# zifeo/distributed-sgd

Hardware: NVIDIA H100
Metric: sgd_samples_per_sec (higher is better)
Workload: dtype f64

## Files before the change

### distributed_sgd_b200/csrc/dsgd_api.cu

```cuda
#include "../../include/dsgd.h"

#include <cuda.h>
#include <cuda_runtime.h>
#include <dlfcn.h>
#include <nccl.h>

#include <algorithm>
#include <cmath>
#include <cstdarg>
#include <cstdio>
#include <cstring>
#include <limits>
#include <mutex>
#include <string>
#include <type_traits>
#include <utility>
#include <vector>

#include "dsgd_kernels.cuh"
#include "dsgd_persistent.cuh"
#include "dsgd_stream.cuh"
#include "dsgd_async.cuh"
#include "dsgd_metrics.cuh"
#include "dsgd_calibrate.cuh"
// ... 91 lines not shown
  dev_buf<float> yabs;
  dev_buf<double> sw;

  dev_buf<double> w, g, d, w_req;
  dev_buf<float> w32, w32_req;
  dev_buf<unsigned long long> n_exact;
  bool stream_ready = false;
  dev_buf<double> scal;
  dev_buf<unsigned long long> cnt;
  dev_buf<double> partial;
  dev_buf<double> out2;
  dev_buf<double> cls_out;
  dev_buf<double> gsum;
  std::vector<int32_t> worker_counts;
  int32_t n_local = 1, k_total = 0;
  bool have_d = false;

  dev_buf<int32_t> samples;
  int64_t samples_n = 0;
  dev_buf<double> losses;
  dev_buf<double> lrs;
  dev_buf<double> preds;
  dev_buf<int32_t> eval_ids;
  dev_buf<unsigned long long> m_keys, m_alt, m_cnt;
  dev_buf<unsigned char> m_tmp;
  dev_buf<double> m_val, m_valt;
  dev_buf<limb_sum> c_pre;
  dev_buf<unsigned long long> c_cnt, c_merged;
  dev_buf<int> c_excl;
  dev_buf<double> c_thr;
  dev_buf<long long> c_tp, c_fp;
  dev_buf<double> k_score, k_cw;
  dev_buf<int8_t> k_lab;
  dev_buf<unsigned long long> k_ctl, k_eval;
  int k_fit_occ = 0;
  int k_fit_occ_w = 0;
  dev_buf<int> i_hull;
  dev_buf<u256> i_wpt;
  dev_buf<int> i_wkeep;
  dev_buf<double> i_wthr, i_wblk;
  dev_buf<double> i_out, i_map;
  dev_buf<long long> i_blk;
  dev_buf<unsigned long long> i_ctl;

  ncclComm_t comm = nullptr;

  dev_buf<double> p_wbuf[2];
  dev_buf<double> p_gbuf[3];
  dev_buf<double2> p_rec[3];
  dev_buf<unsigned long long> p_acc;
  dev_buf<unsigned> p_hinge;
  dev_buf<unsigned long long> p_hcode;
  dev_buf<double> p_loss_nrm;
  dev_buf<unsigned> p_bar;
  bool p_ready = false;
  dev_buf<long long> p_tl;

  dev_buf<double> avg;
  bool avg_on = false;
  int64_t avg_n = 0;

  owned_stream astream;
  owned_stream stream2;
  dev_buf<double> m_w;
  dev_buf<double> outbox;
  peer_ptr peer_w[kMaxReplicas];
  dev_buf<int> a_stop;
  dev_buf<unsigned long long> a_cnt;
  dev_buf<double> a_scratch;
  dev_buf<int32_t> a_rows, a_assigned, a_replay;
  dev_buf<int32_t> u_idx; dev_buf<double> u_val;
  std::mutex u_mu;
  bool a_running = false;
  owned_event a_ev0, a_ev1;

  dev_buf<double> xblk;
  peer_ptr peer_x[kMaxWorld];
  int grid_limit = 0;
  int64_t x_step = 0;
  int64_t x_steps_run = 0;
  dev_buf<unsigned long long> x_llw;
  dev_buf<unsigned long long> x_stats;

  int32_t prof_every = 0;
  int64_t prof_seen = 0;
  std::vector<std::pair<owned_event, owned_event>> prof_events;
  size_t prof_used = 0;

  mutable std::string err;
  mutable std::string info;
};

static thread_local std::string g_create_err;

struct nccl_api {
  ncclResult_t (*GetUniqueId)(ncclUniqueId *) = nullptr;
  ncclResult_t (*CommInitRank)(ncclComm_t *, int, ncclUniqueId, int) = nullptr;
  ncclResult_t (*AllReduce)(const void *, void *, size_t, ncclDataType_t, ncclRedOp_t, ncclComm_t, cudaStream_t) = nullptr;
  ncclResult_t (*CommDestroy)(ncclComm_t) = nullptr;
  const char *(*GetErrorString)(ncclResult_t) = nullptr;
  bool ok = false;
  std::string why;
};
static nccl_api &nccl() {
  static nccl_api api = [] {
    nccl_api a;
// ... 1943 lines not shown
  memcpy(id, &u, sizeof u);
  return DSGD_OK;
}

extern "C" int dsgd_comm_init(dsgd_ctx *ctx, const uint8_t id[DSGD_UNIQUE_ID_BYTES]) {
  if (!ctx) return DSGD_ERR_INVALID;
  NEED(id, DSGD_ERR_INVALID, "dsgd_comm_init: id is NULL");
  NEED(!ctx->comm, DSGD_ERR_STATE, "dsgd_comm_init: communicator already initialised");
  CU(cudaSetDevice(ctx->device));
  ncclUniqueId u;
  memcpy(&u, id, sizeof u);
  NEED(nccl().ok, DSGD_ERR_NCCL, "%s", nccl().why.c_str());
  NC(nccl().CommInitRank(&ctx->comm, ctx->world, u, ctx->rank));
  return DSGD_OK;
}

constexpr int kPCons = 8, kPUpd = 6, kPStages = 8, kPStagePairs = 2560, kPMaxChunks = 128;
using PSmem = PersistSmem<kPCons, kPUpd, kPStages, kPStagePairs, kPMaxChunks>;
constexpr int kPersistForms = 28, kPersistFused = 24;
constexpr bool pf_multi(int f) { return f >= kPersistFused; }
constexpr int pf_weight(int f) { return pf_multi(f) ? kUnweighted : f / 8; }
constexpr bool pf_l1(int f) { return (f & 4) != 0; }
template <int... F>
static void *const *persist_forms(std::integer_sequence<int, F...>) {
  static void *const k[] = {(void *)k_sync_persistent<kPCons, kPUpd, kPStages, kPStagePairs, kPMaxChunks, pf_multi(F),
                                                      (F & 2) != 0, (F & 1) != 0, pf_l1(F), pf_weight(F)>...};
  return k;
}
static void *const *const kPersistKernels = persist_forms(std::make_integer_sequence<int, kPersistForms>{});
static int persist_form(bool multi, bool avg, bool lr_table, bool l1, int weight) {
  if (multi) return kPersistFused + 2 * avg + lr_table;
  return 8 * weight + 4 * l1 + 2 * avg + lr_table;
}
static size_t persist_smem(int f) {
  return sizeof(PSmem) + (pf_weight(f) == kSampleWeighted ? sizeof(PersistSwSmem<kPStages>) : 0);
}
static bool persist_timeline() { static const bool v = getenv("DSGD_PERSIST_TIMELINE") != nullptr; return v; }

static int persist_prepare(dsgd_ctx *ctx, int64_t n_steps) {
  if (!ctx->p_ready) {
    const int64_t nv = (int64_t)ctx->dim + 2;
    const size_t vd = sizeof(double) * (size_t)nv;
    for (int i = 0; i < 2; ++i) CU(ctx->p_wbuf[i].alloc(nv));
    for (int i = 0; i < 3; ++i) {
      CU(ctx->p_gbuf[i].alloc(nv));
      CU(cudaMemsetAsync(ctx->p_gbuf[i], 0, vd, ctx->stream));
      CU(ctx->p_rec[i].alloc(nv));
      CU(cudaMemsetAsync(ctx->p_rec[i], 0, 2 * vd, ctx->stream));
    }
    CU(ctx->p_acc.alloc(3 * kAccStride));
    CU(ctx->p_bar.alloc(4));
    for (int f = 0; f < kPersistForms; ++f)
      CU(cudaFuncSetAttribute(kPersistKernels[f], cudaFuncAttributeMaxDynamicSharedMemorySize, (int)persist_smem(f)));
    ctx->p_ready = true;
  }
  int rc = ctx->p_hinge.grow(ctx, (int64_t)ctx->sm_count * n_steps, 4096 * (int64_t)ctx->sm_count);
  if (rc) return rc;
  if (weighting(ctx) == kSampleWeighted &&
      (rc = ctx->p_hcode.grow(ctx, (int64_t)ctx->sm_count * n_steps, 4096 * (int64_t)ctx->sm_count)))
    return rc;
  return ctx->p_loss_nrm.grow(ctx, 2 * n_steps, 2 * 4096);
}

static int persist_grid(const dsgd_ctx *ctx, int64_t batch) {
  const int g = ctx->grid_limit > 0 ? std::min(ctx->grid_limit, ctx->sm_count) : ctx->sm_count;
  if (cdiv(batch, kMaxRowsPerCta) > g) return 0;
  if (ctx->n_pairs >= (1ll << 31)) return 0;
  return g;
}
static bool persist_multi_fits(const dsgd_ctx *ctx, int G) {
  const int slice = (cdiv(ctx->dim + 1, G) + 31) & ~31;
  return slice <= (kPCons + kPUpd) * 32;
}

static cudaError_t persist_launch(dsgd_ctx *ctx, int form, int G, void **args) {
  void *fn = kPersistKernels[form];
  const size_t smem = persist_smem(form);
  if (ctx->grid_limit > 0) return cudaLaunchKernel(fn, dim3(G), dim3((kPCons + kPUpd + 1) * 32), args, smem, ctx->stream);
  return cudaLaunchCooperativeKernel(fn, dim3(G), dim3((kPCons + kPUpd + 1) * 32), args, smem, ctx->stream);
}

static size_t xblk_stride(const dsgd_ctx *ctx) { return (size_t)(ctx->dim + kReplicaPad); }
static size_t xblk_words(const dsgd_ctx *ctx) { return ((size_t)ctx->dim + 1 + 31) / 32; }
static size_t xblk_bm_offset(const dsgd_ctx *ctx) { return 2 * (size_t)kMaxWorld * 2 * xblk_stride(ctx); }
static size_t xblk_doubles(const dsgd_ctx *ctx) { return xblk_bm_offset(ctx) + (size_t)kMaxWorld * 2 * xblk_words(ctx); }

static int xblk_ensure(dsgd_ctx *ctx) {
  if (ctx->xblk) return DSGD_OK;
  CU(cudaSetDevice(ctx->device));
  CU(ctx->xblk.alloc((int64_t)xblk_doubles(ctx)));
  CU(cudaMemset(ctx->xblk, 0, sizeof(double) * xblk_doubles(ctx)));
  CU(ctx->x_stats.alloc(4));
  CU(cudaMemset(ctx->x_stats, 0, sizeof(unsigned long long) * 4));
  return DSGD_OK;
}

static int xllw_ensure(dsgd_ctx *ctx) {
  if (ctx->x_llw) return DSGD_OK;
  CU(ctx->x_llw.alloc(2 * 2 * (int64_t)xblk_stride(ctx)));
  CU(cudaMemsetAsync(ctx->x_llw, 0, 2 * 2 * sizeof(unsigned long long) * xblk_stride(ctx), ctx->stream));
  return DSGD_OK;
}

static bool xchg_complete(const dsgd_ctx *ctx) {
  if (ctx->world <= 1 || ctx->world > kMaxWorld || !ctx->xblk) return false;
  for (int r = 0; r < ctx->world; ++r)
    if (r != ctx->rank && !ctx->peer_x[r]) return false;
  return true;
}

static int persist_run(dsgd_ctx *ctx, bool multi, const int32_t *samples_dev, int64_t n_per_step, int64_t n_steps,
                       double lr, const double *lrs_host, double *losses_dev) {
  int rc = persist_prepare(ctx, n_steps);
  if (rc) return rc;
  const int G = persist_grid(ctx, n_per_step);
  NEED((uint64_t)G * (uint64_t)(n_steps + 2) < (1ull << 32), DSGD_ERR_INVALID, "dsgd_sync_steps: too many steps for one launch");
  PersistParams pp;
  memset(&pp, 0, sizeof pp);
  pp.rp16 = ctx->rp16; pp.pairs = ctx->pairs; pp.label = ctx->label; pp.samples = samples_dev;
  pp.n_steps = n_steps; pp.batch = (int32_t)n_per_step; pp.dim = ctx->dim;
  pp.wbuf[0] = ctx->p_wbuf[0]; pp.wbuf[1] = ctx->p_wbuf[1];
  for (int i = 0; i < 3; ++i) { pp.gbuf[i] = ctx->p_gbuf[i]; pp.rec[i] = ctx->p_rec[i]; }
  pp.d = ctx->d; pp.acc = ctx->p_acc; pp.bar = ctx->p_bar; pp.hinge = ctx->p_hinge; pp.losses = losses_dev;
  pp.loss_nrm = ctx->p_loss_nrm;
  pp.w_out = ctx->w; pp.w32_out = ctx->w32; pp.scal = ctx->scal;
  pp.abort_flag = reinterpret_cast<int *>(ctx->p_bar + 1);
  CU(cudaMemsetAsync(ctx->p_acc, 0, sizeof(unsigned long long) * 3 * kAccStride, ctx->stream));
  pp.lambda = ctx->lambda; pp.lr = lr; pp.world = 1;
  CU(cudaMemsetAsync(ctx->p_bar, 0, sizeof(unsigned) * 4, ctx->stream));
  if (persist_timeline()) {
    if (!ctx->p_tl) CU(ctx->p_tl.alloc(kTlWords));
    CU(cudaMemsetAsync(ctx->p_tl, 0, sizeof(long long) * kTlWords, ctx->stream));
    pp.tl = ctx->p_tl;
  }
  if (!multi) {
    k_rec_init<<<cdiv(ctx->dim, 256), 256, 0, ctx->stream>>>(ctx->w, ctx->dim, ctx->p_rec[0], ctx->p_rec[1], ctx->p_rec[2]);
    LAUNCHED();
    pp.k_den = 1.0;
    pp.timeout_cycles = 4000000000ll;
  } else {
    CU(cudaMemcpyAsync(ctx->p_wbuf[0], ctx->w, sizeof(double) * (size_t)ctx->dim, cudaMemcpyDeviceToDevice, ctx->stream));
    pp.k_den = (double)ctx->world;
    pp.timeout_cycles = 20000000000ll;
    pp.world = ctx->world; pp.rank = ctx->rank; pp.step_base = ctx->x_step;
    pp.xstride = (int)xblk_stride(ctx);
    pp.xwords = (int)xblk_words(ctx);
    for (int r = 0; r < ctx->world; ++r) {
      unsigned long long *blk = reinterpret_cast<unsigned long long *>((r == ctx->rank) ? ctx->xblk.p : ctx->peer_x[r].p);
      pp.xval[r] = blk;
      pp.xbm[r] = blk + xblk_bm_offset(ctx);
    }
    if ((rc = xllw_ensure(ctx))) return rc;
    pp.llw[0] = ctx->x_llw;
    pp.llw[1] = ctx->x_llw + 2 * xblk_stride(ctx);
    pp.xstats = ctx->x_stats;
  }
  if (ctx->avg_on) pp.avg = ctx->avg;
  if (lrs_host) {
    if ((rc = ctx->lrs.grow(ctx, n_steps, 1024))) return rc;
    CU(cudaMemcpyAsync(ctx->lrs, lrs_host, sizeof(double) * (size_t)n_steps, cudaMemcpyHostToDevice, ctx->stream));
    pp.lrs = ctx->lrs;
    pp.lr = 0.0;
  }
  void *args[] = {&pp};
  const bool l1 = !multi && ctx->lambda1 > 0.0;
  pp.lambda1 = l1 ? ctx->lambda1 : 0.0;
  pp.w_pos = ctx->cw_pos; pp.w_neg = ctx->cw_neg;
  const int weight = multi ? kUnweighted : weighting(ctx);
  if (weight == kSampleWeighted) { pp.sw = ctx->sw; pp.hcode = ctx->p_hcode; }
  const int form = persist_form(multi, ctx->avg_on, lrs_host != nullptr, l1, weight);
  cudaError_t launch_err = cudaSuccess;
  profiled(ctx, [&] { launch_err = persist_launch(ctx, form, G, args); });
  CU(launch_err);
  LAUNCHED();
  if (ctx->avg_on) ctx->avg_n += n_steps;
  if (multi) {
    ctx->x_step += n_steps + 6;
    ctx->x_steps_run += n_steps;
  }
  return DSGD_OK;
}

extern "C" int dsgd_reserve(dsgd_ctx *ctx, int64_t n_samples, int64_t n_steps) {
  if (!ctx) return DSGD_ERR_INVALID;
  NEED(n_samples >= 0 && n_steps >= 0, DSGD_ERR_INVALID, "dsgd_reserve: negative size");
  CU(cudaSetDevice(ctx->device));
  int rc = ctx->samples.grow(ctx, n_samples, 1024);
  if (rc) return rc;
  if ((rc = ctx->losses.grow(ctx, n_steps, 1024))) return rc;
  if ((rc = ctx->lrs.grow(ctx, n_steps, 1024))) return rc;
// ... 679 lines not shown
```

### distributed_sgd_b200/csrc/dsgd_persistent.cuh

```cuda
#pragma once
#include <cuda_runtime.h>
#include <stdint.h>

#include <type_traits>

#include "dsgd_fixed.cuh"
#include "dsgd_kernels.cuh"

namespace dsgd {

constexpr int kMaxWorld = 8;

struct PersistParams {
  const uint32_t *rp16;
  const uint2 *pairs;
  const int8_t *label;
  const int32_t *samples;
  int64_t n_steps;
  int32_t batch;
  int32_t dim;
  double *wbuf[2];
  double *gbuf[3];
  double2 *rec[3];
  const double *d;
  unsigned long long *acc;
  unsigned *hinge;
  double *losses;
  double *w_out;
  float *w32_out;
  double *scal;
  unsigned *bar;
  int *abort_flag;
  double lambda, lr, k_den;
  long long timeout_cycles;
  long long *tl;
  int world, rank;
  int64_t step_base;
  unsigned long long *xval[kMaxWorld];
  unsigned long long *xbm[kMaxWorld];
  int xstride, xwords;
  unsigned long long *llw[2];
  unsigned long long *xstats;
  double *avg;
  const double *lrs;
  double lambda1;
  double *loss_nrm;
  double w_pos, w_neg;
  const double *sw;
  unsigned long long *hcode;
};
static_assert(sizeof(PersistParams) <= 4000, "kernel parameter space is 4 KB");

__device__ __forceinline__ uint32_t smem_u32(const void *p) { return (uint32_t)__cvta_generic_to_shared(p); }
__device__ __forceinline__ void mbar_init(uint64_t *b, unsigned count) {
  asm volatile("mbarrier.init.shared::cta.b64 [%0], %1;" ::"r"(smem_u32(b)), "r"(count) : "memory");
}
__device__ __forceinline__ void mbar_expect_tx(uint64_t *b, unsigned bytes) {
  asm volatile("mbarrier.arrive.expect_tx.shared::cta.b64 _, [%0], %1;" ::"r"(smem_u32(b)), "r"(bytes) : "memory");
}
__device__ __forceinline__ void mbar_arrive(uint64_t *b) {
  asm volatile("mbarrier.arrive.shared::cta.b64 _, [%0];" ::"r"(smem_u32(b)) : "memory");
}
__device__ __forceinline__ void bulk_g2s(void *dst, const void *src, unsigned bytes, uint64_t *b) {
  asm volatile("cp.async.bulk.shared::cluster.global.mbarrier::complete_tx::bytes [%0], [%1], %2, [%3];" ::"r"(
                   smem_u32(dst)),
               "l"(src), "r"(bytes), "r"(smem_u32(b))
               : "memory");
}
__device__ __forceinline__ bool mbar_try_wait(uint64_t *b, unsigned parity) {
  unsigned ok;
  asm volatile(
      "{\n\t.reg .pred p;\n\tmbarrier.try_wait.parity.shared::cta.b64 p, [%1], %2;\n\tselp.u32 %0, 1, 0, p;\n\t}"
      : "=r"(ok)
      : "r"(smem_u32(b)), "r"(parity)
      : "memory");
  return ok != 0;
}
__device__ __forceinline__ void mbar_wait(uint64_t *b, unsigned parity, int *abort_flag, long long timeout) {
  if (mbar_try_wait(b, parity)) return;
  const long long t0 = clock64();
  unsigned spins = 0;
  while (!mbar_try_wait(b, parity)) {
    if ((++spins & 255u) == 0u && (clock64() - t0 > timeout || *(volatile int *)abort_flag)) {
      *(volatile int *)abort_flag = 1;
      return;
    }
  }
}
__device__ __forceinline__ unsigned ld_relaxed_gpu(const unsigned *p) {
  unsigned v;
  asm volatile("ld.relaxed.gpu.global.u32 %0, [%1];" : "=r"(v) : "l"(p) : "memory");
  return v;
}
__device__ __forceinline__ void red_release_gpu_add(unsigned *p, unsigned v) {
  asm volatile("red.release.gpu.global.add.u32 [%0], %1;" ::"l"(p), "r"(v) : "memory");
}
__device__ __forceinline__ unsigned atom_acq_rel_gpu_add(unsigned *p, unsigned v) {
  unsigned old;
  asm volatile("atom.acq_rel.gpu.global.add.u32 %0, [%1], %2;" : "=r"(old) : "l"(p), "r"(v) : "memory");
  return old;
}
__device__ __forceinline__ void st_relaxed_gpu(unsigned *p, unsigned v) {
// ... 18 lines not shown
  const unsigned long long w1 = (bits >> 32) | ((unsigned long long)tag << 32);
  asm volatile("st.relaxed.sys.global.v2.u64 [%0], {%1, %2};" ::"l"(dst), "l"(w0), "l"(w1) : "memory");
}
__device__ __forceinline__ bool ll_try_load(const unsigned long long *src, unsigned tag, double &v) {
  unsigned long long w0, w1;
  asm volatile("ld.relaxed.sys.global.v2.u64 {%0, %1}, [%2];" : "=l"(w0), "=l"(w1) : "l"(src) : "memory");
  if ((unsigned)(w0 >> 32) != tag || (unsigned)(w1 >> 32) != tag) return false;
  v = __longlong_as_double((long long)((w0 & 0xffffffffull) | (w1 << 32)));
  return true;
}
__device__ __forceinline__ void ll_store32(unsigned long long *dst, unsigned v, unsigned tag) {
  const unsigned long long w = (unsigned long long)v | ((unsigned long long)tag << 32);
  asm volatile("st.relaxed.sys.global.u64 [%0], %1;" ::"l"(dst), "l"(w) : "memory");
}
__device__ __forceinline__ bool ll_try_load32(const unsigned long long *src, unsigned tag, unsigned &v) {
  unsigned long long w;
  asm volatile("ld.relaxed.sys.global.u64 %0, [%1];" : "=l"(w) : "l"(src) : "memory");
  v = (unsigned)w;
  return (unsigned)(w >> 32) == tag;
}

__device__ __forceinline__ double apply_update(double wv, double graw, double c, bool add_c, double k_den, double lr) {
  double v = filt(graw);
  if (v != 0.0) {
    if (add_c) v = filt(v + c);
    if (v != 0.0) {
      const double mean = (k_den == 1.0) ? v : filt(v / k_den);
      const double step = filt(mean * lr);
      wv = filt(wv - step);
    }
  }
  return wv;
}

__device__ __forceinline__ bool grid_barrier_arrive_wait(unsigned *bar, unsigned target, int *abort_flag, long long timeout) {
  red_release_gpu_add(bar, 1u);
  const long long t0 = clock64();
  unsigned spins = 0;
  bool ok = true;
  while ((int)(ld_relaxed_gpu(bar) - target) < 0) {
    if ((++spins & 1023u) == 0u && (clock64() - t0 > timeout || *(volatile int *)abort_flag)) {
      *(volatile int *)abort_flag = 1;
      ok = false;
      break;
    }
  }
  return ok;
}

constexpr int kChunkPairs = 128;
static_assert(kChunkPairs == kFoldPairs, "a listed row's chunks are the chunks of the row fold");
constexpr uint32_t kChunkGlobal = 1u << 31;
constexpr int kMaxRowsPerCta = 32;
constexpr int kRowBarFirst = 5, kRowBars = 11;

template <int kMaxChunks>
struct StageMeta {
  int n_rows;
  int n_chunks;
  int n_multi;
  int two_pass;
  int n_pairs;
  int row_y[kMaxRowsPerCta];
  uint32_t row_b[kMaxRowsPerCta];
  int row_len[kMaxRowsPerCta];
  short row_first[kMaxRowsPerCta];
  short row_nch[kMaxRowsPerCta];
  signed char row_bar[kMaxRowsPerCta];
  uint32_t ch_off[kMaxChunks];
  short ch_n[kMaxChunks];
  short ch_row[kMaxChunks];
  double part[kMaxChunks];
};

template <int kStages>
struct PersistSwSmem {
  double row_c[kStages][kMaxRowsPerCta];
  unsigned long long code;
};

template <int kCons, int kUpd, int kStages, int kStagePairs, int kMaxChunks>
struct PersistSmem {
  uint2 ring[kStages][kStagePairs];
  StageMeta<kMaxChunks> meta[kStages];
  uint64_t full[kStages];
  uint64_t empty[kStages];
  uint64_t c_bar[2];
  uint64_t u_bar;
  double red[kCons + kUpd][2];
  double c_val[2];
  double nrm_val[2];
  unsigned hinge_acc;
  int ok;
  long long tl_warp[kCons + kUpd];
};

#define DSGD_TL(slot_)                                                                        \
  do {                                                                                        \
    if (p.tl && blockIdx.x == 0 && lane == 0 && t < 256) p.tl[t * 16 + (slot_)] = clock64(); \
  } while (0)
constexpr int kTlSteps = 4, kTlFirst = 100, kTlCtas = 160, kTlPerCta = 4;
constexpr int kTlWords = 256 * 16 + kTlSteps * kTlCtas * kTlPerCta;

template <bool kL1 = false>
struct FetchLocal {
  const double2 *R;
  uint64_t *cbar;
  unsigned cpar;
  const double *cval;
  int *abort_flag;
  long long timeout;
  double k_den, lr;
  double tau = 0.0;
  double c = 0.0;
  bool add_c = false, have_c = false, good = true;
  __device__ __forceinline__ void need_c() {
    if (!have_c) {
      mbar_wait(cbar, cpar, abort_flag, timeout);
      c = *(volatile const double *)cval;
      add_c = (c != 0.0) && (fabs(c) > kEps);
      have_c = true;
// ... 55 lines not shown
        w0[u] = 0ull; w1[u] = 0ull;
        if (pend & (1u << u))
          asm volatile("ld.relaxed.sys.global.v2.u64 {%0, %1}, [%2];" : "=l"(w0[u]), "=l"(w1[u]) : "l"(LW + 2 * (size_t)pr[u].x) : "memory");
      }
#pragma unroll
      for (int u = 0; u < 4; ++u)
        if ((pend & (1u << u)) && (unsigned)(w0[u] >> 32) == tag && (unsigned)(w1[u] >> 32) == tag) {
          wv[u] = __longlong_as_double((long long)((w0[u] & 0xffffffffull) | (w1[u] << 32)));
          pend &= ~(1u << u);
        }
      if (pend && (++spins & 63u) == 0u && (clock64() - t0 > timeout || *(volatile int *)abort_flag)) {
        *(volatile int *)abort_flag = 1;
        good = false;
        pend = 0;
      }
    }
  }
  __device__ __forceinline__ double get1(uint32_t col) {
    double v;
    spin(LW + 2 * (size_t)col, v);
    return v;
  }
};

template <int kMaxChunks>
__device__ __forceinline__ void chunk_pairs(const StageMeta<kMaxChunks> &mt, const uint2 *ring, const uint2 *pairs, int c, int lane,
                                            uint2 (&pr)[4]) {
  const uint32_t off = mt.ch_off[c];
  const int n = mt.ch_n[c];
  const uint2 *src = (off & kChunkGlobal) ? (pairs + (off & ~kChunkGlobal)) : (ring + off);
#pragma unroll
  for (int u = 0; u < 4; ++u) {
    const int k = u * 32 + lane;
    pr[u] = (k < n) ? src[k] : make_uint2(0u, 0u);
  }
}

template <int kCons, int kMaxChunks, int kWeight = kUnweighted, class Fetch>
__device__ __forceinline__ std::conditional_t<kWeight == kSampleWeighted, unsigned long long, unsigned> consume_stage(
    StageMeta<kMaxChunks> &mt, const uint2 *ring, const uint2 *pairs, double *gbase, const int gstride, Fetch &fetch, int warp,
    int lane, long long *tl, const uint2 (*pre)[4] = nullptr, double w_pos = 1.0, double w_neg = 1.0,
    const double *row_c = nullptr) {
  using Hinge = std::conditional_t<kWeight == kSampleWeighted, unsigned long long, unsigned>;
  const int n_ch = mt.n_chunks;
  Hinge hinge = 0;
  auto scale_of = [&](int yi, double y, int m) {
    if constexpr (kWeight == kSampleWeighted) return yi > 0 ? row_c[m] : -row_c[m];
    return kWeight == kClassWeighted ? (yi > 0 ? w_pos : -w_neg) : y;
  };
  auto hinge_of = [&](int yi, unsigned l, int m) -> Hinge {
    if constexpr (kWeight == kSampleWeighted) return (Hinge)l << (2 * m);
    return kWeight == kClassWeighted ? l << (yi > 0 ? 0 : 16) : l;
  };
  for (int c = warp; c < n_ch; c += kCons) {
    uint2 pr[4];
    double wv[4];
    if (pre && c == warp) {
#pragma unroll
      for (int u = 0; u < 4; ++u) pr[u] = (*pre)[u];
    } else {
      chunk_pairs(mt, ring, pairs, c, lane, pr);
    }
    fetch.get4(pr, wv);
    double acc = 0.0;
#pragma unroll
    for (int u = 0; u < 4; ++u) acc += filt(filt((double)__uint_as_float(pr[u].y)) * wv[u]);
    if (tl && lane == 0 && c == warp) tl[2] = clock64();
    acc = warp_sum(acc);
    if (tl && lane == 0 && c == warp) tl[4] = clock64();
    {
      const int row1 = mt.ch_row[c];
      const int nch1 = mt.row_nch[row1];
      int first1 = c;
      if (nch1 > 1) {
        if (lane == 0) mt.part[c] = acc;
        const int bar = mt.row_bar[row1];
        if (bar < 0) continue;
        named_bar_sync(bar, nch1 * 32);
        first1 = mt.row_first[row1];
        acc = 0.0;
        for (int i = 0; i < nch1; ++i) acc += mt.part[first1 + i];
      }
      {
        const int yi = mt.row_y[row1];
        const double y = (double)yi;
        if (c == first1 && lane == 0) hinge += hinge_of(yi, (unsigned)(1 - yi * pred_of(acc)), row1);
        if (!(y * acc < 0.0)) {
          const double sc = scale_of(yi, y, row1);
#pragma unroll
          for (int u = 0; u < 4; ++u) {
            const double gvv = filt(filt((double)__uint_as_float(pr[u].y)) * sc);
            if (gvv != 0.0) red_add_f64(gbase + (size_t)gstride * pr[u].x, gvv);
          }
        }
      }
    }
  }
  if (mt.two_pass) {
    named_bar_sync(2, kCons * 32);
    for (int c = warp; c < n_ch; c += kCons) {
      const int row = mt.ch_row[c];
      const int first = mt.row_first[row], nch = mt.row_nch[row];
      if (nch == 1) continue;
      double dot = 0.0;
      for (int i = 0; i < nch; ++i) dot += mt.part[first + i];
      const int yi = mt.row_y[row];
      const double y = (double)yi;
      if (c == first && lane == 0) hinge += hinge_of(yi, (unsigned)(1 - yi * pred_of(dot)), row);
      if (!(y * dot < 0.0)) {
        const double sc = scale_of(yi, y, row);
        const uint32_t off = mt.ch_off[c];
        const int n = mt.ch_n[c];
        const uint2 *src = (off & kChunkGlobal) ? (pairs + (off & ~kChunkGlobal)) : (ring + off);
        for (int k = lane; k < n; k += 32) {
          const uint2 pr = src[k];
          const double gvv = filt(filt((double)__uint_as_float(pr.y)) * sc);
          if (gvv != 0.0) red_add_f64(gbase + (size_t)gstride * pr.x, gvv);
        }
      }
    }
  }
  for (int m = warp; m < mt.n_rows; m += kCons) {
    const int nch = mt.row_nch[m];
    if (nch == 0) {
      if (lane == 0) hinge += hinge_of(mt.row_y[m], 1u, m);
    } else if (nch < 0) {
      const uint2 *grow = pairs + (size_t)mt.row_b[m] * 2;
      const int len = mt.row_len[m];
      const double dot = row_fold(grow, 0, len, lane, [&](uint32_t c) { return fetch.get1(c); });
      const int yi = mt.row_y[m];
      const double y = (double)yi;
      if (lane == 0) hinge += hinge_of(yi, (unsigned)(1 - yi * pred_of(dot)), m);
      if (!(y * dot < 0.0))
        for (int k = lane; k < len; k += 32) {
          const uint2 pr = __ldg(&grow[k]);
          const double gvv = filt(filt((double)__uint_as_float(pr.y)) * scale_of(yi, y, m));
          if (gvv != 0.0) red_add_f64(gbase + (size_t)gstride * pr.x, gvv);
        }
    }
  }
  return hinge;
}

template <int kCons, int kUpd, int kStages, int kStagePairs, int kMaxChunks, bool kMulti, bool kAvg, bool kLrTable,
          bool kL1 = false, int kWeight = kUnweighted>
__global__ void __launch_bounds__((kCons + kUpd + 1) * 32, 1) k_sync_persistent(const PersistParams p) {
  using Smem = PersistSmem<kCons, kUpd, kStages, kStagePairs, kMaxChunks>;
  static_assert(!kL1 || (!kMulti && kUpd <= kCons), "the L1 form is one-GPU only and keeps its partials in the consumers' slots");
  static_assert(kWeight == kUnweighted || !kMulti, "the weighted forms are one-GPU only");
  static_assert(2 * kMaxRowsPerCta <= 64, "a CTA's hinge codes of one step fit one 64-bit word");
  static_assert(2 * kMaxRowsPerCta < (1 << 16), "a CTA's hinge count of one class fits a 16-bit half");
  static_assert(kAccWords + kAccLimbs <= kAccStride, "the L1 limbs follow the accumulator's overflow word");
  static_assert(kCons / 2 <= kRowBars, "every row of several chunks in a stage of at most kCons chunks has a named barrier");
  extern __shared__ __align__(128) unsigned char smem_raw[];
  Smem &sm = *reinterpret_cast<Smem *>(smem_raw);
  using SwSmem = PersistSwSmem<kStages>;
  SwSmem &swm = *reinterpret_cast<SwSmem *>(smem_raw + sizeof(Smem));

  const int lane = threadIdx.x & 31;
  const int warp = threadIdx.x >> 5;
  const bool is_cons = warp < kCons;
  const bool is_upd = warp >= kCons && warp < kCons + kUpd;
  const int G = gridDim.x;
  const int B = p.batch;
  const int64_t S = p.n_steps;
  constexpr int kSyncThreads = (kCons + kUpd) * 32;
  const int n_r = (B > (int)blockIdx.x) ? (B - 1 - (int)blockIdx.x) / G + 1 : 0;

  if (threadIdx.x == 0) {
    for (int s = 0; s < kStages; ++s) {
      mbar_init(&sm.full[s], 1u);
      mbar_init(&sm.empty[s], (unsigned)kCons);
    }
    mbar_init(&sm.c_bar[0], 1u);
    mbar_init(&sm.c_bar[1], 1u);
    mbar_init(&sm.u_bar, (unsigned)(kMulti ? kCons + kUpd : kUpd));
    sm.c_val[0] = 0.0;
    sm.nrm_val[0] = 0.0;
    sm.hinge_acc = 0u;
    if constexpr (kWeight == kSampleWeighted) swm.code = 0ull;
    sm.ok = 1;
  }
  asm volatile("fence.mbarrier_init.release.cluster;" ::: "memory");
  __syncthreads();
  if (threadIdx.x == 0) mbar_arrive(&sm.c_bar[0]);

  if (!is_cons && !is_upd) {
    auto load_id = [&](int64_t t) -> int32_t {
      return (t < S && lane < n_r) ? __ldg(&p.samples[t * B + blockIdx.x + lane * G]) : -1;
    };
    uint32_t b0 = 0, e0 = 0, b1 = 0, e1 = 0;
    int y0 = 0, y1 = 0;
    double s0 = 0.0, s1 = 0.0;
    auto load_win = [&](int32_t id, uint32_t &b, uint32_t &e, int &y, double &sw) {
      b = 0u; e = 0u; y = 0;
      if constexpr (kWeight == kSampleWeighted) sw = 0.0;
      if (id >= 0) {
        b = __ldg(&p.rp16[id]);
        e = __ldg(&p.rp16[id + 1]);
        y = (int)__ldg(&p.label[id]);
        if constexpr (kWeight == kSampleWeighted) sw = __ldg(&p.sw[id]);
      }
    };
    load_win(load_id(0), b0, e0, y0, s0);
    load_win(load_id(1), b1, e1, y1, s1);
    int32_t id_next = load_id(2);
    for (int64_t t = 0; t < S; ++t) {
      const int st = (int)t & (kStages - 1);
      if (t >= kStages) {
        mbar_wait(&sm.empty[st], (unsigned)(((t / kStages) - 1) & 1), p.abort_flag, p.timeout_cycles);
        if (*(volatile int *)p.abort_flag) return;
      }
      auto &mt = sm.meta[st];
      const int len = (lane < n_r) ? (int)(e0 - b0) * 2 : 0;
      const int nch = (len + kChunkPairs - 1) / kChunkPairs;
      int ps = len, cs = nch;
#pragma unroll
      for (int o = 1; o < 32; o <<= 1) {
        const int a = __shfl_up_sync(0xffffffffu, ps, o), c2 = __shfl_up_sync(0xffffffffu, cs, o);
        if (lane >= o) { ps += a; cs += c2; }
      }
      const int my_pair = ps - len, my_chunk = cs - nch;
      const bool listed = (my_chunk + nch) <= kMaxChunks;
      const bool in_ring = listed && (my_pair + len) <= kStagePairs;
      if (lane < n_r) {
        mt.row_y[lane] = y0;
        if constexpr (kWeight == kSampleWeighted) swm.row_c[st][lane] = (y0 > 0 ? p.w_pos : p.w_neg) * s0;
        mt.row_b[lane] = b0;
        mt.row_len[lane] = len;
        mt.row_first[lane] = (short)my_chunk;
        mt.row_nch[lane] = (short)(listed ? nch : -1);
        if (listed) {
          for (int c = 0; c < nch; ++c) {
            const int n = min(kChunkPairs, len - c * kChunkPairs);
            mt.ch_off[my_chunk + c] = in_ring ? (uint32_t)(my_pair + c * kChunkPairs)
                                              : (kChunkGlobal | (b0 * 2u + (uint32_t)(c * kChunkPairs)));
            mt.ch_n[my_chunk + c] = (short)n;
            mt.ch_row[my_chunk + c] = (short)lane;
          }
        }
      }
      const unsigned my_bytes = (lane < n_r && in_ring) ? (unsigned)len * 8u : 0u;
      const unsigned ring_bytes = __reduce_add_sync(0xffffffffu, my_bytes);
      const int listed_chunks = __reduce_max_sync(0xffffffffu, (lane < n_r && listed) ? (my_chunk + nch) : 0);
      const unsigned multi = __ballot_sync(0xffffffffu, lane < n_r && listed && nch > 1);
      const bool per_row = __all_sync(0xffffffffu, lane >= n_r || listed) && listed_chunks <= kCons;
      if (lane < n_r)
        mt.row_bar[lane] = (signed char)((per_row && nch > 1) ? kRowBarFirst + __popc(multi & ((1u << lane) - 1u)) : -1);
      if (lane == 31) mt.n_pairs = ps;
      if (lane == 0) {
        mt.n_rows = n_r;
        mt.n_chunks = listed_chunks;
        mt.n_multi = __popc(multi);
        mt.two_pass = (multi != 0u && !per_row) ? 1 : 0;
      }
      __syncwarp();
      if (lane == 0) {
        if (ring_bytes) mbar_expect_tx(&sm.full[st], ring_bytes);
        else mbar_arrive(&sm.full[st]);
      }
      __syncwarp();
      if (my_bytes) bulk_g2s(&sm.ring[st][my_pair], p.pairs + (size_t)b0 * 2, my_bytes, &sm.full[st]);
      b0 = b1; e0 = e1; y0 = y1;
      if constexpr (kWeight == kSampleWeighted) s0 = s1;
      load_win(id_next, b1, e1, y1, s1);
      id_next = load_id(t + 3);
    }
    return;
  }

  double lr = p.lr;
  const int64_t base = kMulti ? p.step_base : 0;
  unsigned phase = 0;
  const int n_upd = G * kUpd * 32;
  const int u0 = blockIdx.x * kUpd * 32 + ((int)threadIdx.x - kCons * 32);
  const int K = p.world, me = p.rank;
  const int slice = ((p.dim + 1 + G - 1) / G + 31) & ~31;
  const int j_col = blockIdx.x * slice + (int)threadIdx.x;
  const bool col_act = kMulti && (int)threadIdx.x < slice && j_col <= p.dim;
  const int col_word = j_col >> 5;
  unsigned long long st_val = 0, st_bm = 0;
  constexpr int kUpdCols = 2;
  double wreg[kUpdCols], dreg[kUpdCols];
  double areg[kUpdCols];
  int ttl[kUpdCols];
  bool gnz[kUpdCols];
#pragma unroll
  for (int i = 0; i < kUpdCols; ++i) {
    wreg[i] = dreg[i] = 0.0;
    areg[i] = 0.0;
    ttl[i] = 0;
    gnz[i] = false;
    if constexpr (!kMulti) {
      const int j = u0 + i * n_upd;
      if (is_upd && j < p.dim) {
        wreg[i] = __ldcg(&p.rec[2][j].x);
        dreg[i] = __ldg(&p.d[j]);
        if constexpr (kAvg) areg[i] = p.avg[j];
      }
    }
  }
  if constexpr (kMulti) {
    if (col_act && j_col < p.dim) {
      wreg[0] = __ldcg(&p.wbuf[0][j_col]);
      dreg[0] = __ldg(&p.d[j_col]);
      if constexpr (kAvg) areg[0] = p.avg[j_col];
    }
  }

  uint2 pre[4];
  auto prefetch = [&](int64_t tn) {
    const int st = (int)tn & (kStages - 1);
    const auto &mt = sm.meta[st];
    mbar_wait(&sm.full[st], (unsigned)(((unsigned)tn / kStages) & 1u), p.abort_flag, p.timeout_cycles);
#pragma unroll
    for (int u = 0; u < 4; ++u) pre[u] = make_uint2(0u, 0u);
    if (warp < mt.n_chunks) chunk_pairs(mt, &sm.ring[st][0], p.pairs, warp, lane, pre);
  };
  if (!kMulti && is_cons && S > 0) prefetch(0);
// ... 388 lines not shown
            p.losses[s] = pen + (hp_w + hn_w) / (double)B;
          }
        } else {
          for (int b = lane; b < G; b += 32) h += __ldcg(&p.hinge[s * G + b]);
          h = __reduce_add_sync(0xffffffffu, h);
          if (lane == 0) {
            if constexpr (kL1)
              p.losses[s] = p.lambda * __ldcg(&p.loss_nrm[s]) + p.lambda1 * __ldcg(&p.loss_nrm[S + s]) + (double)h / (double)B;
            else
              p.losses[s] = p.lambda * __ldcg(&p.loss_nrm[s]) + (double)h / (double)B;
          }
        }
      }
    }
  }
  if constexpr (kMulti) {
    const unsigned long long *LW = p.llw[(base + S) & 1];
    const unsigned wtag = (unsigned)(base + S + 1);
    const int n_all = G * kSyncThreads;
    for (int j = blockIdx.x * kSyncThreads + threadIdx.x; j < p.dim; j += n_all) {
      double wv = 0.0;
      ll_try_load(LW + 2 * (size_t)j, wtag, wv);
      p.w_out[j] = wv;
      p.w32_out[j] = (float)wv;
    }
    if (p.xstats && lane == 0 && (st_val | st_bm)) {
      atomicAdd(&p.xstats[0], st_val);
      atomicAdd(&p.xstats[1], st_bm);
    }
    if constexpr (kAvg) {
      if (col_act && j_col < p.dim) p.avg[j_col] = areg[0];
    }
  } else if (is_upd) {
    const double2 *Rfin = p.rec[ti_prev];
#pragma unroll
    for (int i = 0; i < kUpdCols; ++i) {
      const int j = u0 + i * n_upd;
      if (j < p.dim) {
        p.w_out[j] = wreg[i];
        p.w32_out[j] = (float)wreg[i];
        if constexpr (kAvg) p.avg[j] = areg[i];
      }
    }
    for (int j = u0 + kUpdCols * n_upd; j < p.dim; j += n_upd) {
      const double wv = __ldcg(&Rfin[j]).x;
      p.w_out[j] = wv;
      p.w32_out[j] = (float)wv;
    }
  }
  if constexpr (kWeight == kSampleWeighted) {
    if (p.losses) {
      for (int64_t s = (int64_t)blockIdx.x * (kCons + kUpd) + warp; s < S; s += (int64_t)G * (kCons + kUpd)) {
        unsigned long long lim[kLossLimbs] = {0, 0, 0, 0, 0, 0}, ovf = 0;
        for (int i = lane; i < B; i += 32) {
          const int b = i % G, m = i / G;
          const unsigned code = (unsigned)(__ldcg(&p.hcode[s * G + b]) >> (2 * m)) & 3u;
          const int32_t id = __ldg(&p.samples[s * B + i]);
          const double c = (__ldg(&p.label[id]) > 0 ? p.w_pos : p.w_neg) * __ldg(&p.sw[id]);
          acc_add_local(lim, ovf, c * (double)code);
        }
#pragma unroll
        for (int o = 16; o > 0; o >>= 1) {
#pragma unroll
          for (int k = 0; k < kLossLimbs; ++k) lim[k] += __shfl_xor_sync(0xffffffffu, lim[k], o);
          ovf += __shfl_xor_sync(0xffffffffu, ovf, o);
        }
        if (lane == 0) {
          unsigned long long q[kLossAccWords];
#pragma unroll
          for (int k = 0; k < kLossLimbs; ++k) q[k] = lim[k];
          q[kLossLimbs] = ovf;
          double pen = p.lambda * __ldcg(&p.loss_nrm[s]);
          if constexpr (kL1) pen = pen + p.lambda1 * __ldcg(&p.loss_nrm[S + s]);
          p.losses[s] = pen + acc_value(q) / (double)B;
        }
      }
    }
  }
}

__global__ void __launch_bounds__(256) k_rec_init(const double *__restrict__ w, int dim, double2 *__restrict__ rec0,
                                                  double2 *__restrict__ rec1, double2 *__restrict__ rec2) {
  const int j = blockIdx.x * blockDim.x + threadIdx.x;
  if (j < dim) {
    const double2 r = make_double2(w[j], 0.0);
    rec0[j] = r;
    rec1[j] = r;
    rec2[j] = r;
  }
}

}
```

Measured before the change: 76.19 million.

## Precompute per-step load-balanced row placement plan with multi-chunk row splitting across CTAs

Adds a pre-pass kernel, fused into the record-init launch, that for every step assigns sample rows to CTAs greedily by chunk load. When there is spare capacity it also splits long rows across two CTAs, with only one of them counting the hinge loss. The producer warp of the persistent kernel reads this plan instead of using a fixed strided row assignment. The aim is to balance per-CTA work and cut tail latency from long rows. The cost is an extra plan kernel with serial warp-level placement per step, more plan memory traffic, and one full dot product computed redundantly for each split row.

```diff
diff --git a/distributed_sgd_b200/csrc/dsgd_api.cu b/distributed_sgd_b200/csrc/dsgd_api.cu
--- a/distributed_sgd_b200/csrc/dsgd_api.cu
+++ b/distributed_sgd_b200/csrc/dsgd_api.cu
@@ -167,6 +167,8 @@
   dev_buf<unsigned> p_hinge;
   dev_buf<unsigned long long> p_hcode;
   dev_buf<double> p_loss_nrm;
+  dev_buf<int> p_plan_off;
+  dev_buf<uint2> p_plan;
   dev_buf<unsigned> p_bar;
   bool p_ready = false;
   dev_buf<long long> p_tl;
@@ -2216,6 +2218,8 @@
     CU(ctx->p_bar.alloc(4));
     for (int f = 0; f < kPersistForms; ++f)
       CU(cudaFuncSetAttribute(kPersistKernels[f], cudaFuncAttributeMaxDynamicSharedMemorySize, (int)persist_smem(f)));
+    CU(cudaFuncSetAttribute(k_rec_init_plan, cudaFuncAttributeMaxDynamicSharedMemorySize,
+                            (int)plan_smem_bytes(ctx->sm_count, kMaxRowsPerCta * ctx->sm_count)));
     ctx->p_ready = true;
   }
   int rc = ctx->p_hinge.grow(ctx, (int64_t)ctx->sm_count * n_steps, 4096 * (int64_t)ctx->sm_count);
@@ -2230,6 +2234,7 @@
   const int g = ctx->grid_limit > 0 ? std::min(ctx->grid_limit, ctx->sm_count) : ctx->sm_count;
   if (cdiv(batch, kMaxRowsPerCta) > g) return 0;
   if (ctx->n_pairs >= (1ll << 31)) return 0;
+  if (g > 255) return 0;
   return g;
 }
 static bool persist_multi_fits(const dsgd_ctx *ctx, int G) {
@@ -2298,8 +2303,14 @@
     pp.tl = ctx->p_tl;
   }
   if (!multi) {
-    k_rec_init<<<cdiv(ctx->dim, 256), 256, 0, ctx->stream>>>(ctx->w, ctx->dim, ctx->p_rec[0], ctx->p_rec[1], ctx->p_rec[2]);
+    const int B = (int)n_per_step, stride = std::min(2 * B, kMaxRowsPerCta * G), n_rec = cdiv(ctx->dim, 32);
+    if ((rc = ctx->p_plan_off.grow(ctx, n_steps * (G + 1), 4096 * (int64_t)(G + 1)))) return rc;
+    if ((rc = ctx->p_plan.grow(ctx, n_steps * stride, 4096 * (int64_t)stride))) return rc;
+    k_rec_init_plan<<<n_rec + (int)n_steps, 32, plan_smem_bytes(G, B), ctx->stream>>>(
+        ctx->w, ctx->dim, ctx->p_rec[0], ctx->p_rec[1], ctx->p_rec[2], n_rec, samples_dev, ctx->rp16, B, G, stride,
+        ctx->p_plan_off, ctx->p_plan);
     LAUNCHED();
+    pp.plan_off = ctx->p_plan_off; pp.plan = ctx->p_plan; pp.plan_stride = stride;
     pp.k_den = 1.0;
     pp.timeout_cycles = 4000000000ll;
   } else {
diff --git a/distributed_sgd_b200/csrc/dsgd_persistent.cuh b/distributed_sgd_b200/csrc/dsgd_persistent.cuh
--- a/distributed_sgd_b200/csrc/dsgd_persistent.cuh
+++ b/distributed_sgd_b200/csrc/dsgd_persistent.cuh
@@ -48,6 +48,9 @@
   double w_pos, w_neg;
   const double *sw;
   unsigned long long *hcode;
+  const int *plan_off;
+  const uint2 *plan;
+  int plan_stride;
 };
 static_assert(sizeof(PersistParams) <= 4000, "kernel parameter space is 4 KB");
 
@@ -172,6 +175,9 @@
 static_assert(kChunkPairs == kFoldPairs, "a listed row's chunks are the chunks of the row fold");
 constexpr uint32_t kChunkGlobal = 1u << 31;
 constexpr int kMaxRowsPerCta = 32;
+constexpr int kSplitAbove = 2;
+constexpr uint32_t kFullRow = 0xffff0000u;
+constexpr int kSplitRowsPerCta = 4;
 constexpr int kRowBarFirst = 5, kRowBars = 11;
 
 template <int kMaxChunks>
@@ -187,6 +193,7 @@
   short row_first[kMaxRowsPerCta];
   short row_nch[kMaxRowsPerCta];
   signed char row_bar[kMaxRowsPerCta];
+  uint32_t row_sc[kMaxRowsPerCta];
   uint32_t ch_off[kMaxChunks];
   short ch_n[kMaxChunks];
   short ch_row[kMaxChunks];
@@ -348,6 +355,11 @@
     if constexpr (kWeight == kSampleWeighted) return (Hinge)l << (2 * m);
     return kWeight == kClassWeighted ? l << (yi > 0 ? 0 : 16) : l;
   };
+  auto scatters = [&](int m, int k) {
+    const uint32_t sc = mt.row_sc[m];
+    return k >= (int)(sc & 0xffffu) && k < (int)(sc >> 16);
+  };
+  auto counts = [&](int m) { return (mt.row_sc[m] & 0xffffu) == 0u; };
   for (int c = warp; c < n_ch; c += kCons) {
     uint2 pr[4];
     double wv[4];
@@ -380,8 +392,8 @@
       {
         const int yi = mt.row_y[row1];
         const double y = (double)yi;
-        if (c == first1 && lane == 0) hinge += hinge_of(yi, (unsigned)(1 - yi * pred_of(acc)), row1);
-        if (!(y * acc < 0.0)) {
+        if (c == first1 && lane == 0 && counts(row1)) hinge += hinge_of(yi, (unsigned)(1 - yi * pred_of(acc)), row1);
+        if (!(y * acc < 0.0) && scatters(row1, c - first1)) {
           const double sc = scale_of(yi, y, row1);
 #pragma unroll
           for (int u = 0; u < 4; ++u) {
@@ -402,8 +414,8 @@
       for (int i = 0; i < nch; ++i) dot += mt.part[first + i];
       const int yi = mt.row_y[row];
       const double y = (double)yi;
-      if (c == first && lane == 0) hinge += hinge_of(yi, (unsigned)(1 - yi * pred_of(dot)), row);
-      if (!(y * dot < 0.0)) {
+      if (c == first && lane == 0 && counts(row)) hinge += hinge_of(yi, (unsigned)(1 - yi * pred_of(dot)), row);
+      if (!(y * dot < 0.0) && scatters(row, c - first)) {
         const double sc = scale_of(yi, y, row);
         const uint32_t off = mt.ch_off[c];
         const int n = mt.ch_n[c];
@@ -426,9 +438,11 @@
       const double dot = row_fold(grow, 0, len, lane, [&](uint32_t c) { return fetch.get1(c); });
       const int yi = mt.row_y[m];
       const double y = (double)yi;
-      if (lane == 0) hinge += hinge_of(yi, (unsigned)(1 - yi * pred_of(dot)), m);
+      if (lane == 0 && counts(m)) hinge += hinge_of(yi, (unsigned)(1 - yi * pred_of(dot)), m);
+      const uint32_t sc = mt.row_sc[m];
+      const int lo = (int)(sc & 0xffffu) * kChunkPairs, hi = sc == kFullRow ? len : min(len, (int)(sc >> 16) * kChunkPairs);
       if (!(y * dot < 0.0))
-        for (int k = lane; k < len; k += 32) {
+        for (int k = lo + lane; k < hi; k += 32) {
           const uint2 pr = __ldg(&grow[k]);
           const double gvv = filt(filt((double)__uint_as_float(pr.y)) * scale_of(yi, y, m));
           if (gvv != 0.0) red_add_f64(gbase + (size_t)gstride * pr.x, gvv);
@@ -482,25 +496,36 @@
   if (threadIdx.x == 0) mbar_arrive(&sm.c_bar[0]);
 
   if (!is_cons && !is_upd) {
-    auto load_id = [&](int64_t t) -> int32_t {
-      return (t < S && lane < n_r) ? __ldg(&p.samples[t * B + blockIdx.x + lane * G]) : -1;
+    auto load_ent = [&](int64_t t) -> uint2 {
+      if constexpr (kMulti) {
+        return (t < S && lane < n_r) ? make_uint2((uint32_t)__ldg(&p.samples[t * B + blockIdx.x + lane * G]), kFullRow)
+                                     : make_uint2(~0u, 0u);
+      } else {
+        if (t >= S) return make_uint2(~0u, 0u);
+        const int *o = p.plan_off + t * (G + 1) + blockIdx.x;
+        const int a = __ldg(&o[0]);
+        return lane < __ldg(&o[1]) - a ? __ldg(&p.plan[t * p.plan_stride + a + lane]) : make_uint2(~0u, 0u);
+      }
     };
     uint32_t b0 = 0, e0 = 0, b1 = 0, e1 = 0;
+    uint32_t r0 = 0, r1 = 0;
     int y0 = 0, y1 = 0;
     double s0 = 0.0, s1 = 0.0;
-    auto load_win = [&](int32_t id, uint32_t &b, uint32_t &e, int &y, double &sw) {
+    auto load_win = [&](uint2 ent, uint32_t &b, uint32_t &e, int &y, double &sw, uint32_t &r) {
       b = 0u; e = 0u; y = 0;
+      r = ent.y;
       if constexpr (kWeight == kSampleWeighted) sw = 0.0;
-      if (id >= 0) {
+      if (r != 0u) {
+        const int32_t id = (int32_t)ent.x;
         b = __ldg(&p.rp16[id]);
         e = __ldg(&p.rp16[id + 1]);
         y = (int)__ldg(&p.label[id]);
         if constexpr (kWeight == kSampleWeighted) sw = __ldg(&p.sw[id]);
       }
     };
-    load_win(load_id(0), b0, e0, y0, s0);
-    load_win(load_id(1), b1, e1, y1, s1);
-    int32_t id_next = load_id(2);
+    load_win(load_ent(0), b0, e0, y0, s0, r0);
+    load_win(load_ent(1), b1, e1, y1, s1, r1);
+    uint2 ent_next = load_ent(2);
     for (int64_t t = 0; t < S; ++t) {
       const int st = (int)t & (kStages - 1);
       if (t >= kStages) {
@@ -508,7 +533,8 @@
         if (*(volatile int *)p.abort_flag) return;
       }
       auto &mt = sm.meta[st];
-      const int len = (lane < n_r) ? (int)(e0 - b0) * 2 : 0;
+      const bool mine = r0 != 0u;
+      const int len = mine ? (int)(e0 - b0) * 2 : 0;
       const int nch = (len + kChunkPairs - 1) / kChunkPairs;
       int ps = len, cs = nch;
 #pragma unroll
@@ -519,8 +545,9 @@
       const int my_pair = ps - len, my_chunk = cs - nch;
       const bool listed = (my_chunk + nch) <= kMaxChunks;
       const bool in_ring = listed && (my_pair + len) <= kStagePairs;
-      if (lane < n_r) {
+      if (mine) {
         mt.row_y[lane] = y0;
+        mt.row_sc[lane] = r0;
         if constexpr (kWeight == kSampleWeighted) swm.row_c[st][lane] = (y0 > 0 ? p.w_pos : p.w_neg) * s0;
         mt.row_b[lane] = b0;
         mt.row_len[lane] = len;
@@ -536,16 +563,17 @@
           }
         }
       }
-      const unsigned my_bytes = (lane < n_r && in_ring) ? (unsigned)len * 8u : 0u;
+      const unsigned my_bytes = (mine && in_ring) ? (unsigned)len * 8u : 0u;
       const unsigned ring_bytes = __reduce_add_sync(0xffffffffu, my_bytes);
-      const int listed_chunks = __reduce_max_sync(0xffffffffu, (lane < n_r && listed) ? (my_chunk + nch) : 0);
-      const unsigned multi = __ballot_sync(0xffffffffu, lane < n_r && listed && nch > 1);
-      const bool per_row = __all_sync(0xffffffffu, lane >= n_r || listed) && listed_chunks <= kCons;
-      if (lane < n_r)
+      const int listed_chunks = __reduce_max_sync(0xffffffffu, (mine && listed) ? (my_chunk + nch) : 0);
+      const unsigned multi = __ballot_sync(0xffffffffu, mine && listed && nch > 1);
+      const bool per_row = __all_sync(0xffffffffu, !mine || listed) && listed_chunks <= kCons;
+      if (mine)
         mt.row_bar[lane] = (signed char)((per_row && nch > 1) ? kRowBarFirst + __popc(multi & ((1u << lane) - 1u)) : -1);
+      const int n_rows = __popc(__ballot_sync(0xffffffffu, mine));
       if (lane == 31) mt.n_pairs = ps;
       if (lane == 0) {
-        mt.n_rows = n_r;
+        mt.n_rows = n_rows;
         mt.n_chunks = listed_chunks;
         mt.n_multi = __popc(multi);
         mt.two_pass = (multi != 0u && !per_row) ? 1 : 0;
@@ -557,10 +585,10 @@
       }
       __syncwarp();
       if (my_bytes) bulk_g2s(&sm.ring[st][my_pair], p.pairs + (size_t)b0 * 2, my_bytes, &sm.full[st]);
-      b0 = b1; e0 = e1; y0 = y1;
+      b0 = b1; e0 = e1; y0 = y1; r0 = r1;
       if constexpr (kWeight == kSampleWeighted) s0 = s1;
-      load_win(id_next, b1, e1, y1, s1);
-      id_next = load_id(t + 3);
+      load_win(ent_next, b1, e1, y1, s1, r1);
+      ent_next = load_ent(t + 3);
     }
     return;
   }
@@ -1055,12 +1083,17 @@
     if (p.losses) {
       for (int64_t s = (int64_t)blockIdx.x * (kCons + kUpd) + warp; s < S; s += (int64_t)G * (kCons + kUpd)) {
         unsigned long long lim[kLossLimbs] = {0, 0, 0, 0, 0, 0}, ovf = 0;
-        for (int i = lane; i < B; i += 32) {
-          const int b = i % G, m = i / G;
-          const unsigned code = (unsigned)(__ldcg(&p.hcode[s * G + b]) >> (2 * m)) & 3u;
-          const int32_t id = __ldg(&p.samples[s * B + i]);
-          const double c = (__ldg(&p.label[id]) > 0 ? p.w_pos : p.w_neg) * __ldg(&p.sw[id]);
-          acc_add_local(lim, ovf, c * (double)code);
+        const int *o = p.plan_off + s * (G + 1);
+        for (int b = lane; b < G; b += 32) {
+          const int a = __ldg(&o[b]), n = __ldg(&o[b + 1]) - a;
+          const unsigned long long codes = __ldcg(&p.hcode[s * G + b]);
+          for (int m = 0; m < n; ++m) {
+            const unsigned code = (unsigned)(codes >> (2 * m)) & 3u;
+            if (code == 0u) continue;
+            const int32_t id = (int32_t)__ldg(&p.plan[s * p.plan_stride + a + m]).x;
+            const double c = (__ldg(&p.label[id]) > 0 ? p.w_pos : p.w_neg) * __ldg(&p.sw[id]);
+            acc_add_local(lim, ovf, c * (double)code);
+          }
         }
 #pragma unroll
         for (int o = 16; o > 0; o >>= 1) {
@@ -1082,15 +1115,122 @@
   }
 }
 
-__global__ void __launch_bounds__(256) k_rec_init(const double *__restrict__ w, int dim, double2 *__restrict__ rec0,
-                                                  double2 *__restrict__ rec1, double2 *__restrict__ rec2) {
-  const int j = blockIdx.x * blockDim.x + threadIdx.x;
-  if (j < dim) {
-    const double2 r = make_double2(w[j], 0.0);
-    rec0[j] = r;
-    rec1[j] = r;
-    rec2[j] = r;
-  }
-}
-
-}
+__host__ __device__ constexpr size_t plan_smem_bytes(int G, int B) { return sizeof(int) * (2 * (size_t)G + 3 * (size_t)B); }
+__global__ void __launch_bounds__(32) k_rec_init_plan(const double *__restrict__ w, int dim, double2 *__restrict__ rec0,
+                                                      double2 *__restrict__ rec1, double2 *__restrict__ rec2, int n_rec,
+                                                      const int32_t *__restrict__ samples, const uint32_t *__restrict__ rp16,
+                                                      int B, int G, int stride, int *__restrict__ plan_off,
+                                                      uint2 *__restrict__ plan) {
+  const int lane = threadIdx.x;
+  if ((int)blockIdx.x < n_rec) {
+    const int j = blockIdx.x * 32 + lane;
+    if (j < dim) {
+      const double2 r = make_double2(w[j], 0.0);
+      rec0[j] = r;
+      rec1[j] = r;
+      rec2[j] = r;
+    }
+    return;
+  }
+  const int64_t t = (int64_t)blockIdx.x - n_rec;
+  const int32_t *ids = samples + t * B;
+  extern __shared__ int plan_sm[];
+  int *load = plan_sm, *cnt = load + G;
+  uint32_t *place = (uint32_t *)(cnt + G);
+  uint32_t *key = place + B, *sorted = key + B;
+  __shared__ int n_multi;
+  constexpr uint32_t kOne = 0xfffffffeu, kEmpty = 0xfffffffdu;
+  auto nch_of = [&](int i) {
+    const int32_t id = ids[i];
+    return (int)(((rp16[id + 1] - rp16[id]) * 2u + kChunkPairs - 1) / kChunkPairs);
+  };
+  for (int b = lane; b < G; b += 32) load[b] = cnt[b] = 0;
+  if (lane == 0) n_multi = 0;
+  __syncwarp();
+  for (int i = lane; i < B; i += 32) {
+    const int n = nch_of(i);
+    place[i] = n == 0 ? kEmpty : kOne;
+    if (n > 1) key[atomicAdd(&n_multi, 1)] = (uint32_t)min(n, 0x7fff) << 16 | (uint32_t)(0xffff - i);
+  }
+  __syncwarp();
+  const int M = n_multi;
+  for (int j = lane; j < M; j += 32) {
+    const uint32_t kj = key[j];
+    int r = 0;
+    for (int k = 0; k < M; ++k) r += key[k] > kj;
+    sorted[r] = kj;
+  }
+  __syncwarp();
+  auto put = [&](int nch, int avoid) -> uint32_t {
+    unsigned best = ~0u, any = ~0u;
+    for (int b = lane; b < G; b += 32)
+      if (cnt[b] < kMaxRowsPerCta) {
+        const unsigned k = (unsigned)load[b] << 8 | (unsigned)b;
+        any = min(any, k);
+        if (b != avoid) best = min(best, k);
+      }
+    best = __reduce_min_sync(0xffffffffu, best);
+    if (best == ~0u) best = __reduce_min_sync(0xffffffffu, any);
+    const int b = (int)(best & 0xffu);
+    const int slot = cnt[b];
+    __syncwarp();
+    if (lane == 0) { cnt[b] = slot + 1; load[b] += nch; }
+    __syncwarp();
+    return (uint32_t)b | (uint32_t)slot << 8;
+  };
+  int splits = (G > 1 && B <= kSplitRowsPerCta * G) ? kMaxRowsPerCta * G - B : 0;
+  for (int r = 0; r < M; ++r) {
+    const uint32_t k = sorted[r];
+    const int i = 0xffff - (int)(k & 0xffffu), n = (int)(k >> 16);
+    const uint32_t a = put(n, -1);
+    uint32_t pl = a | 0xffff0000u;
+    if (n > kSplitAbove && n < 0x7fff && splits > 0) {
+      pl = a | put(n, (int)(a & 0xffu)) << 16;
+      --splits;
+    }
+    if (lane == 0) place[i] = pl;
+    __syncwarp();
+  }
+  for (int pass = 0; pass < 2; ++pass) {
+    const uint32_t want = pass == 0 ? kOne : kEmpty;
+    for (int i = 0; i < B; ++i)
+      if (place[i] == want) {
+        const uint32_t a = put(pass == 0 ? 1 : 0, -1);
+        if (lane == 0) place[i] = a | 0xffff0000u;
+        __syncwarp();
+      }
+  }
+  int run = 0;
+  int *off = plan_off + t * (G + 1);
+  for (int b0 = 0; b0 < G; b0 += 32) {
+    const int b = b0 + lane;
+    const int c = b < G ? cnt[b] : 0;
+    int s = c;
+#pragma unroll
+    for (int o = 1; o < 32; o <<= 1) {
+      const int v = __shfl_up_sync(0xffffffffu, s, o);
+      if (lane >= o) s += v;
+    }
+    if (b < G) {
+      off[b] = run + s - c;
+      load[b] = run + s - c;
+    }
+    run += __shfl_sync(0xffffffffu, s, 31);
+  }
+  if (lane == 0) off[G] = run;
+  __syncwarp();
+  uint2 *ent = plan + t * stride;
+  for (int i = lane; i < B; i += 32) {
+    const uint32_t pl = place[i], lo = pl & 0xffffu, hi = pl >> 16;
+    const uint32_t id = (uint32_t)ids[i];
+    if (hi == 0xffffu) {
+      ent[load[lo & 0xffu] + (lo >> 8)] = make_uint2(id, kFullRow);
+    } else {
+      const uint32_t n = (uint32_t)nch_of(i), h = (n + 1) / 2;
+      ent[load[lo & 0xffu] + (lo >> 8)] = make_uint2(id, h << 16);
+      ent[load[hi & 0xffu] + (hi >> 8)] = make_uint2(id, h | n << 16);
+    }
+  }
+}
+
+}
```

Measured after the change: 75.67 million, median of 6. No clear change (-0.7%).
